# n-lalanne/LDSO

Hardware: AMD Instinct MI355X
Metric: point-residuals/sec per GN iter (7-KF window) + ms/solve; 1/2/4/8 GPU (higher is better)
Workload: dtype f32

## Files before the change

### include/ldso_ba.h

```cpp
#ifndef LDSO_BA_H_
#define LDSO_BA_H_

#include <stddef.h>
#include <stdint.h>

#ifdef __cplusplus
extern "C" {
#endif

#define LDSO_BA_ABI_VERSION 6

#define LDSO_BA_PATTERN_NUM 8
#define LDSO_BA_CPARS 4
#define LDSO_BA_MAX_FRAMES 16
#define LDSO_BA_PRECALC_STRIDE 48
#define LDSO_BA_POINT_STRIDE 24

#define LDSO_BA_RES_IN 0
#define LDSO_BA_RES_OOB 1
#define LDSO_BA_RES_OUTLIER 2

#define LDSO_BA_FLAG_ACTIVE 1u
#define LDSO_BA_FLAG_NEW 2u

// ... 196 lines not shown

int ldso_ba_frame_step(int32_t n_frames, const ldso_ba_frame_state *in, const double *x, ldso_ba_frame_state *out,
                       double *calib_value, const double *calib_value_zero, float *calib_scaled_out,
                       float *c_delta_out);

int ldso_ba_step_canbreak(int32_t n_frames, const double *x, float sum_nid, float num_id, float th_opt_iterations,
                          int32_t *canbreak_out);

int ldso_ba_set_kernel_timing(ldso_ba_ctx *ctx, int32_t enable);

#define LDSO_BA_TUNE_TILED_IMAGES 2
#define LDSO_BA_TUNE_TOP_CHUNK 6
#define LDSO_BA_TUNE_TIMING_MASK 7
#define LDSO_BA_TUNE_ITEM_ORDER 10
#define LDSO_BA_TUNE_SOLVE_EXACT 12
int ldso_ba_set_tuning(ldso_ba_ctx *ctx, int32_t key, int32_t value);
int ldso_ba_get_kernel_times(ldso_ba_ctx *ctx, double *ms, int64_t *counts, int32_t n);
const char *ldso_ba_kernel_name(int32_t i);
int32_t ldso_ba_num_kernels(void);

int ldso_ba_stats(ldso_ba_ctx *ctx, int64_t *device_bytes, int64_t *n_points,
                  int64_t *n_residuals);

#ifdef __cplusplus
}
#endif

#endif
```

### ldso_amd/_lib.py

```python
from __future__ import annotations

import ctypes as C
import os

import numpy as np

HERE = os.path.dirname(os.path.abspath(__file__))
LIB_DIR = os.path.join(HERE, "lib")
LIB_PATH = os.environ.get("LDSO_BA_LIB") or os.path.join(LIB_DIR, "libldso_ba.so")
SYNTH_PATH = os.path.join(LIB_DIR, "libldso_synth.so")

PATTERN_NUM = 8
CPARS = 4
MAX_FRAMES = 16
PRECALC_STRIDE = 48
POINT_STRIDE = 24
RES_IN, RES_OOB, RES_OUTLIER = 0, 1, 2
FLAG_ACTIVE, FLAG_NEW = 1, 2

i32p = C.POINTER(C.c_int32)
f32p = C.POINTER(C.c_float)
f64p = C.POINTER(C.c_double)
i8p = C.POINTER(C.c_int8)
u8p = C.POINTER(C.c_uint8)
# ... 144 lines not shown
    ("ldso_ba_comm_init", C.c_int, [C.c_void_p, C.c_void_p, C.c_int32, C.c_int32]),
    ("ldso_ba_check_settings", C.c_int, [C.c_void_p]),
    ("ldso_ba_default_settings", None, [C.c_void_p]),
    ("ldso_ba_set_settings", C.c_int, [C.c_void_p, C.c_void_p]),
    ("ldso_ba_get_settings", C.c_int, [C.c_void_p, C.c_void_p]),
    ("ldso_ba_optimize", C.c_int, [C.c_void_p, C.c_int32, C.c_void_p, C.c_void_p, f64p, f64p, f64p, f64p, C.c_void_p,
                                   f64p, f32p, i32p, i32p]),
    ("ldso_ba_frame_step", C.c_int, [C.c_int32, C.c_void_p, f64p, C.c_void_p, f64p, f64p, f32p, f32p]),
    ("ldso_ba_step_canbreak", C.c_int, [C.c_int32, f64p, C.c_float, C.c_float, C.c_float, i32p]),
    ("ldso_ba_set_kernel_timing", C.c_int, [C.c_void_p, C.c_int32]),
    ("ldso_ba_set_tuning", C.c_int, [C.c_void_p, C.c_int32, C.c_int32]),
    ("ldso_ba_get_kernel_times", C.c_int, [C.c_void_p, f64p, i64p, C.c_int32]),
    ("ldso_ba_kernel_name", C.c_char_p, [C.c_int32]),
    ("ldso_ba_num_kernels", C.c_int32, []),
    ("ldso_ba_stats", C.c_int, [C.c_void_p, i64p, i64p, i64p]),
    ("ldso_ba_marginalize_frame", C.c_int, [C.c_int32, C.c_int32, f64p, f64p, f64p, f64p, f64p, f64p]),
    ("ldso_ba_ad_ht_delta", C.c_int, [C.c_int32, f64p, f64p, f64p, f32p]),
    ("ldso_ba_calc_m_energy", C.c_int, [C.c_int32, f64p, f64p, f32p, f64p, f64p]),
    ("ldso_ba_calc_l_energy", C.c_int, [C.c_int32, f64p, f64p, f64p, f32p, C.c_int32, f32p, f32p, f64p]),
    ("ldso_ba_load_marginalization", C.c_int, [C.c_void_p, C.c_void_p, C.c_int32, C.POINTER(LdsoBaWindow)]),
    ("ldso_ba_marginalize_points", C.c_int, [C.c_void_p, f32p, f64p, f64p]),
    ("ldso_ba_activate_points", C.c_int, [C.c_void_p, C.c_int32, C.c_int32, C.c_void_p, C.c_int32, C.c_void_p]),
]

f32pp = C.POINTER(f32p)

IMMATURE_DTYPE = np.dtype([("u", "<f4"), ("v", "<f4"), ("idepth_min", "<f4"), ("idepth_max", "<f4"),
                           ("quality", "<f4"), ("energy_th", "<f4"), ("color", "<f4", (8,)),
                           ("weights", "<f4", (8,)), ("grad_h", "<f4", (4,)), ("host", "<i4"),
                           ("last_status", "<i4"), ("last_uv", "<f4", (2,)), ("last_interval", "<f4"),
# ... 69 lines not shown
```

### ldso_amd/context.py

```python
from __future__ import annotations

import ctypes as C

import numpy as np

from . import _lib as L
from .window import Window


class BAContext:
    def __init__(self, device: int = 0):
        self._lib = L.lib()
        h = C.c_void_p()
        L.check(self._lib.ldso_ba_create(int(device), C.byref(h)))
        self._h = h
        self.windows: list[Window] = []
        self._structs = None

    def close(self):
        if getattr(self, "_h", None) is not None and self._h.value:
            self._lib.ldso_ba_destroy(self._h)
            self._h = None

    def __del__(self):
# ... 188 lines not shown
        L.check(self._lib.ldso_ba_unpack_system(self._h))

    def set_tuning(self, key: int, value: int):
        L.check(self._lib.ldso_ba_set_tuning(self._h, int(key), int(value)))

    def set_kernel_timing(self, on: bool):
        L.check(self._lib.ldso_ba_set_kernel_timing(self._h, int(bool(on))))

    def kernel_times(self) -> dict:
        n = int(self._lib.ldso_ba_num_kernels())
        ms = np.zeros(n, np.float64)
        cnt = np.zeros(n, np.int64)
        L.check(self._lib.ldso_ba_get_kernel_times(self._h, L.ptr(ms, L.f64p), L.ptr(cnt, L.i64p), n))
        return {self._lib.ldso_ba_kernel_name(i).decode(): (float(ms[i]), int(cnt[i])) for i in range(n)}

    def stats(self):
        b, p, r = C.c_int64(), C.c_int64(), C.c_int64()
        L.check(self._lib.ldso_ba_stats(self._h, C.byref(b), C.byref(p), C.byref(r)))
        return dict(device_bytes=b.value, points=p.value, residuals=r.value)
```

### ldso_amd/csrc/ldso_ba.hip

```cpp
#include <hip/hip_runtime.h>
#include <hip/hip_ext.h>
#include <rccl/rccl.h>

#include <algorithm>
#include <atomic>
#include <climits>
#include <cmath>
#include <cstdio>
#include <cstdlib>
#include <cstring>
#include <mutex>
#include <string>
#include <vector>

#include "../../include/ldso_ba.h"
#include "../../include/ldso_ct.h"
#include "ldso_ba_internal.h"
#include "se3.h"

using namespace ldso_ba;

namespace {

constexpr int kWave = 64;
// ... 79 lines not shown
    long long frame_stride;
    int tiles_per_row;
    int fix;
    int accumulate;
    const float *ad_ht_delta;
    const int *stop;
    int pass;
    int aff_fix;
};

struct Geo {
    float Ku, Kv, new_idepth;
    float d_xi_x[6], d_xi_y[6], d_C_x[4], d_C_y[4], d_d_x, d_d_y;
};

__device__ inline bool centre_projection(const float *__restrict__ pre, float u, float v, float idz,
                                         float fxl, float fyl, float cxl, float cyl, float wM3, float hM3,
                                         Geo &g) {
#pragma clang fp contract(off)
    const float fxli = 1.0f / fxl, fyli = 1.0f / fyl;
    const float *R0 = pre + 12, *t0 = pre + 21;
    const float K0 = (u + 0 - cxl) * fxli, K1 = (v + 0 - cyl) * fyli;
    float ptp[3];
#pragma unroll
    for (int i = 0; i < 3; i++) ptp[i] = (R0[3 * i] * K0 + R0[3 * i + 1] * K1 + R0[3 * i + 2] * 1.0f) + t0[i] * idz;
    const float drescale = 1.0f / ptp[2];
    g.new_idepth = idz * drescale;
    if (!(drescale > 0)) return false;
    const float uu = ptp[0] * drescale, vv = ptp[1] * drescale;
    g.Ku = uu * fxl + cxl;
    g.Kv = vv * fyl + cyl;
    if (!(g.Ku > 1.1f && g.Kv > 1.1f && g.Ku < wM3 && g.Kv < hM3)) return false;
    g.d_d_x = drescale * (t0[0] - t0[2] * uu) * kScaleIdepth * fxl;
    g.d_d_y = drescale * (t0[1] - t0[2] * vv) * kScaleIdepth * fyl;
    g.d_C_x[2] = drescale * (R0[6] * uu - R0[0]);
    g.d_C_x[3] = fxl * drescale * (R0[7] * uu - R0[1]) * fyli;
// ... 240 lines not shown
    }
}

typedef float f32x4 __attribute__((ext_vector_type(4)));
constexpr int kTopRow = 36;
constexpr int kTermQ = 9;
constexpr int kBoxCols = 9, kBoxBands = 3, kBoxFloats = 112;
static_assert(kBoxFloats >= (kBoxCols * kBoxBands + 1) * 4, "box");
constexpr int kTermStride = 72;
constexpr int kRoundQ = kTermQ;
static_assert(kTermStride >= kRoundQ * 8, "term tables");
constexpr int kTermsOnly = 8 * kTermStride;
constexpr int kTermsPerWave = 8 * kBoxFloats > kTermsOnly ? 8 * kBoxFloats : kTermsOnly;
constexpr int kSumsPerWave = 64 * kSumStride;

__device__ __forceinline__ void top_mfma(float *tab, int lane, bool active, const Geo &g, const PhotoSums &s,
                                         float *slab_item) {
    auto stage = [&](float4 *row) {
        if (active) {
            row[0] = make_float4(g.d_C_x[0], g.d_C_y[0], g.d_C_x[1], g.d_C_y[1]);
            row[1] = make_float4(g.d_C_x[2], g.d_C_y[2], g.d_C_x[3], g.d_C_y[3]);
            row[2] = make_float4(g.d_xi_x[0], g.d_xi_y[0], g.d_xi_x[1], g.d_xi_y[1]);
            row[3] = make_float4(g.d_xi_x[2], g.d_xi_y[2], g.d_xi_x[3], g.d_xi_y[3]);
            row[4] = make_float4(g.d_xi_x[4], g.d_xi_y[4], g.d_xi_x[5], g.d_xi_y[5]);
            row[5] = make_float4(s.JabJIdx_00, s.JabJIdx_01, s.JabJIdx_10, s.JabJIdx_11);
            row[6] = make_float4(s.JI_r0, s.JI_r1, s.Jab2_00, s.Jab2_11);
            row[7] = make_float4(s.Jab2_01, s.Jab_r1, s.Jab_r0, s.rr);
            row[8] = make_float4(s.JIdx2_00, s.JIdx2_10, s.JIdx2_11, 0.f);
        } else {
            const float4 z = make_float4(0.f, 0.f, 0.f, 0.f);
#pragma unroll
            for (int k = 0; k < 9; k++) row[k] = z;
        }
    };
    const int i = lane & 15, kk = lane >> 4;
    const bool geo = i < 10, ind = i >= 13;
    const float a0c = i == 13 ? 1.f : 0.f, a1c = i == 14 ? 1.f : 0.f;
    stage(reinterpret_cast<float4 *>(tab + lane * kTopRow));
    wave_lds_sync();
    f32x4 acc0 = {0.f, 0.f, 0.f, 0.f}, acc1 = {0.f, 0.f, 0.f, 0.f};
    {
        const float *base = tab + kk * kTopRow;
#pragma unroll 4
        for (int m = 0; m < 16; m += 2) {
#pragma unroll
            for (int u = 0; u < 2; u++) {
                const float *rr = base + 4 * (m + u) * kTopRow;
                const float2 p = *reinterpret_cast<const float2 *>(rr + 2 * i);
                const float4 q = *reinterpret_cast<const float4 *>(rr + 32);
                const float A0 = ind ? a0c : p.x, A1 = ind ? a1c : p.y;
                const float B0 = geo ? q.x * p.x + q.y * p.y : p.x;
                const float B1 = geo ? q.y * p.x + q.z * p.y : p.y;
                f32x4 &acc = u ? acc1 : acc0;
                acc = __builtin_amdgcn_mfma_f32_16x16x4f32(A0, B0, acc, 0, 0, 0);
                acc = __builtin_amdgcn_mfma_f32_16x16x4f32(A1, B1, acc, 0, 0, 0);
            }
        }
    }
    wave_lds_sync();
    const f32x4 acc = acc0 + acc1;
#pragma unroll
    for (int v = 0; v < 4; v++) {
        const int r = 4 * kk + v, c = i;
        int slot = -1;
        if (r < 10 && c < 10 && c >= r) slot = r * 10 - r * (r - 1) / 2 + (c - r);
        else if (r < 10 && c >= 10 && c < 13) slot = 55 + 3 * r + (c - 10);
        else if (r == 13 && c >= 13) slot = 85 + (c - 13);
        else if (r == 14 && c >= 13) slot = 88 + (c - 13);
        if (slot >= 0) slab_item[slot] = acc[v];
        else if (r == 15 && c < 5) slab_item[91 + c] = 0.f;
    }
// ... 13 lines not shown
    v = min(v, LDSO_DPP(v, 0xB1));
    v = min(v, LDSO_DPP(v, 0x4E));
    return min(v, LDSO_DPP(v, 0x141));
}
__device__ __forceinline__ int grp8_or(int v) {
    v |= LDSO_DPP(v, 0xB1);
    v |= LDSO_DPP(v, 0x4E);
    return v | LDSO_DPP(v, 0x141);
}
__device__ __forceinline__ float4 ldb4(__amdgpu_buffer_rsrc_t r, unsigned off) {
    typedef int i32x4 __attribute__((ext_vector_type(4)));
    const i32x4 v = __builtin_bit_cast(i32x4, __builtin_amdgcn_raw_buffer_load_b128(r, (int)off, 0, 0));
    return make_float4(__int_as_float(v.x), __int_as_float(v.y), __int_as_float(v.z), __int_as_float(v.w));
}

template <bool kMarg>
__device__ __forceinline__ void phase_a_pieces(int lane, float *lds_terms_w, float *S, const float *pre, int jlimit,
                                               int my_state, float4 my_pd0, float jp_dx, float jp_dy, float da,
                                               float db, __amdgpu_buffer_rsrc_t rsrc, unsigned band, float wM3,
                                               float hM3, int aff_fix) {
#pragma clang fp contract(off)
    const int g = lane >> 3, sl = lane & 7;
    const bool fixA = (aff_fix & 1) != 0, fixB = (aff_fix & 2) != 0;
    const int px = sl == 1 || sl == 6 ? -1 : sl == 2 ? 1 : sl == 3 ? -2 : sl == 5 ? 2 : 0;
    const int py = sl == 0 ? -2 : sl <= 2 ? -1 : sl <= 5 ? 0 : sl == 6 ? 1 : 2;
    const float aff0 = pre[24], aff1 = pre[25], b0a = pre[26];
    float *T = lds_terms_w + g * kTermStride;
    float *box = lds_terms_w + g * kBoxFloats;
    const int nsteps = (jlimit + 7) >> 3;
    constexpr unsigned kOOB = 0x7FFFFFF0u;

    struct Geo8 {
// ... 141 lines not shown
        step(k, cur, nxt);
        if (k + 1 >= nsteps) break;
        step(k + 1, nxt, cur);
    }
    while (wide_steps) {
        const int k = __builtin_ctz(wide_steps);
        wide_steps &= wide_steps - 1;
        geo(k, cur);
        const bool wide = cur.gok && cur.wide;
        float iv[12];
        if (wide) load12(rsrc, band, (int)cur.Ku, (int)cur.Kv, iv);
        terms(k, cur, wide, iv);
    }
}

template <int kImg, bool kMarg>
__global__ __launch_bounds__(256, kLinBlocksPerCu) void k_linearize(LinParams P) {
    static_assert(kImg == 1 || kImg == 3, "image layouts 1 and 3");
    extern __shared__ __attribute__((aligned(16))) float lds_dyn[];
    const int lane = threadIdx.x & 63;
    const int wave = __builtin_amdgcn_readfirstlane(threadIdx.x >> 6);
    float *lds_terms_w = lds_dyn + wave * kWaveLds;
    float *lds_sums_w = lds_terms_w + kTermsPerWave;
    const int nb = P.n_blocks, xcd = blockIdx.x & 7, q8 = nb >> 3, r8 = nb & 7;
    const int lblock = xcd * q8 + min(xcd, r8) + (blockIdx.x >> 3);
    if (lblock * 4 + wave >= P.n_items) return;
    const int itemL = P.item_base + lblock * 4 + wave;
    const int4 it = P.items[itemL];
    if (P.stop && P.pass > P.stop[__builtin_amdgcn_readfirstlane(it.w)]) return;
    const int cnt = it.y & 0xFFFF;
    const bool valid = lane < cnt;
    const int pair = __builtin_amdgcn_readfirstlane(it.z), jlimit = __builtin_amdgcn_readfirstlane(cnt);
    const WinDev &W = P.wins[__builtin_amdgcn_readfirstlane(it.w)];
    const int N = W.N;
    const int h = (pair - W.pair_base) % N, t = (pair - W.pair_base) / N;
    const float *pre = P.precalc + (size_t)pair * LDSO_BA_PRECALC_STRIDE;
    const float th = fmaxf(P.frame_th[W.frame_base + h], P.frame_th[W.frame_base + t]);
    const float wM3 = W.wM3, hM3 = W.hM3;
    const float4 *img = P.img + (size_t)(W.frame_base + t) * P.frame_stride;
    const __amdgpu_buffer_rsrc_t rsrc = frame_rsrc(reinterpret_cast<const float *>(img), P.frame_stride * 16);
    const unsigned band = (unsigned)P.tiles_per_row * 8u * 16u;

    const int r = it.x + lane;
    const int rq = valid ? r : 0;
    int my_state = P.rs_state[rq];
    const int my_slot = P.rs_slot[rq];
    const int my_point = valid ? W.point_base + (my_slot - W.rec_base - (t < h ? t : t - 1) * W.P) : W.point_base;
    uint8_t flags = P.rs_flags[rq];
    float state_energy = P.rs_energy[rq];
    float new_energy = P.rs_newenergy[rq];
    const float4 my_pd0 = *(const float4 *)(P.pt_data + (size_t)my_point * LDSO_BA_POINT_STRIDE);
    {
        const float4 *cw = reinterpret_cast<const float4 *>(P.pt_data + (size_t)my_point * LDSO_BA_POINT_STRIDE + 8);
        float4 v[4];
#pragma unroll
        for (int u = 0; u < 4; u++) v[u] = cw[u];
        float *row = lds_sums_w + lane * kSumStride;
#pragma unroll
        for (int u = 0; u < 4; u++) {
            row[4 * u] = v[u].x;
            row[4 * u + 1] = v[u].y;
            row[4 * u + 2] = v[u].z;
            row[4 * u + 3] = v[u].w;
        }
    }
    if (!valid) my_state = LDSO_BA_RES_OOB;
    float jp_dx = 0.f, jp_dy = 0.f, da = 0.f, db = 0.f;
    if constexpr (kMarg) {
#pragma clang fp contract(off)
        const float *dp = P.ad_ht_delta + (size_t)pair * 8;
        da = dp[6];
        db = dp[7];
        Geo gm;
        if (centre_projection(pre, my_pd0.x, my_pd0.y, my_pd0.w, W.calib[0], W.calib[1], W.calib[2], W.calib[3],
                              wM3, hM3, gm)) {
            const float dd = P.pt_data[(size_t)my_point * LDSO_BA_POINT_STRIDE + 5];
            float x6 = 0.f, y6 = 0.f, x4 = 0.f, y4 = 0.f;
#pragma unroll
            for (int i = 0; i < 6; i++) {
                x6 += gm.d_xi_x[i] * dp[i];
                y6 += gm.d_xi_y[i] * dp[i];
            }
#pragma unroll
            for (int i = 0; i < 4; i++) {
                x4 += gm.d_C_x[i] * W.cdelta[i];
                y4 += gm.d_C_y[i] * W.cdelta[i];
            }
            jp_dx = x6 + x4 + gm.d_d_x * dd;
            jp_dy = y6 + y4 + gm.d_d_y * dd;
        }
    }
// ... 14 lines not shown
        float *T = lds_terms_w + g * (kTermQ * 8);
        float *S = lds_sums_w;
        const int nsteps = (jlimit + 7) >> 3;
        const int tpr2 = P.tiles_per_row;

        struct Stage {
            float Ku, Kv, color, weight;
            float iv[12];
            float3 t00, t10, t01, t11;
            float jx, jy;
            bool gok;
        };
        auto issue = [&](int k, Stage &q) {
            const int j = 8 * k + g;
            const int st = __shfl(my_state, j, kWave);
            const int p = __shfl(my_point, j, kWave);
            const float pu = __shfl(my_pd0.x, j, kWave), pv = __shfl(my_pd0.y, j, kWave),
                        pz = __shfl(my_pd0.z, j, kWave);
            const bool go = j < jlimit && st != LDSO_BA_RES_OOB;
            if constexpr (kMarg) {
                q.jx = __shfl(jp_dx, j, kWave);
                q.jy = __shfl(jp_dy, j, kWave);
            }
            (void)p;
            q.color = S[j * kSumStride + sl];
            q.weight = S[j * kSumStride + 8 + sl];
            const float up = pu + px, vp = pv + py;
            float ptp[3];
#pragma unroll
            for (int i = 0; i < 3; i++)
                ptp[i] = (pre[3 * i] * up + pre[3 * i + 1] * vp + pre[3 * i + 2] * 1.0f) + pre[9 + i] * pz;
            q.Ku = ptp[0] / ptp[2];
            q.Kv = ptp[1] / ptp[2];
            const bool pok = go && q.Ku > 1.1f && q.Kv > 1.1f && q.Ku < wM3 && q.Kv < hM3;
            const unsigned long long m1 = __ballot(pok);
            q.gok = ((m1 >> (8 * g)) & 0xFFull) == 0xFFull;
            const int ix = pok ? (int)q.Ku : 1, iy = pok ? (int)q.Kv : 1;
            if constexpr (kImg == 3) {
                load12(rsrc, band, ix, iy, q.iv);
// ... 61 lines not shown
            }
            wave_lds_sync();
            if (rok) sum8(kTermQ + sl, sl);
            wave_lds_sync();
        };
        Stage A, B;
        issue(0, A);
        for (int k = 0; k < nsteps; k += 2) {
            issue(k + 1, B);
            consume(k, A);
            issue(k + 2, A);
            consume(k + 1, B);
        }
    }

    double energy = 0;
    bool isIN = false, active = false;
    Geo g;
    PhotoSums s;
    if (valid) {
        const int8_t old_state = (int8_t)my_state;
        int8_t new_state = LDSO_BA_RES_OOB;
        float e_wo = -1;
        if (old_state == LDSO_BA_RES_OOB) {
            energy = state_energy;
            st_nt(P.rec_b + my_slot, make_float2(0.f, __builtin_nanf("")));
        } else {
            const float4 pd0 = my_pd0;
            const float *Sr = lds_sums_w + lane * kSumStride;
            s.energy = Sr[0];
// ... 61 lines not shown
        isIN = (new_state == LDSO_BA_RES_IN);
        st_nt(P.rs_newstate + r, new_state);
        st_nt(P.rs_energy_wo + r, e_wo);
    }

    double esum = energy;
#pragma unroll
    for (int m = 32; m >= 1; m >>= 1) esum += __shfl_xor(esum, m, kWave);
    const unsigned long long inmask = __ballot(isIN);
    if (lane == 0) {
        P.item_energy[2 * itemL] = esum;
        P.item_energy[2 * itemL + 1] = (double)__popcll(inmask);
    }
    if ((it.y >> 16) && P.geo_snap && lane < kGeoSnap)
        P.geo_snap[(size_t)pair * kGeoSnap + lane] = lane < 12 ? pre[12 + lane] : W.calib[lane - 12];
    if (!P.accumulate) return;
    wave_lds_sync();
    top_mfma(lds_terms_w, lane, active, g, s, P.top_slab + (size_t)itemL * kTopVals);
}

struct PointParams {
    const int4 *__restrict__ items;
    const WinDev *__restrict__ wins;
    const float *__restrict__ pt_data;
    const int *__restrict__ pt_nres;
    const unsigned long long *__restrict__ pt_tgt;
    const float4 *__restrict__ rec_a;
    const float2 *__restrict__ rec_b;
    const float *__restrict__ precalc;
    float *pt_out;
    float *sc_slab;
    int n_items;
    int item_base;
// ... 1055 lines not shown
                for (int b = 0; b < 2; b++) {
                    if (r0 + a > c0 + b) continue;
                    o[pk_index(4 + 8 * i + r0 + a, 4 + 8 * i + c0 + b, D)] = v[2 * a + b];
                }
        } else {
            const int item = fu - 16, rr = item < 32 ? item >> 2 : item - 32, cc = item & 3;
            double ha = 0;
            for (int st = 0; st < Nm1; st++) ha += CP[(part * 40 + item) * Nm1 + st];
            if (item < 32)
                (top ? HAp : Hsp)[pk_index(cc, 4 + 8 * i + rr, D)] = ha;
            else
                (top ? bAp : bsp)[4 + 8 * i + rr] = ha;
        }
    }
}
__global__ __launch_bounds__(256) void k_stitch_host_sum(const WinDev *__restrict__ wins,
                                                          const int2 *__restrict__ blocks,
                                                          const double *__restrict__ stage, double *sys) {
    const int2 bw = blocks[blockIdx.x];
    const WinDev &W = wins[bw.x];
    const long long n_el = sys_len(W.D), e = (long long)bw.y + threadIdx.x;
    if (e >= n_el) return;
    const double *p = stage + W.stage_base + e;
    double x[kHostStitchMaxN];
#pragma unroll
    for (int h = 0; h < kHostStitchMaxN; h++) x[h] = p[(size_t)min(h, W.N - 1) * n_el];
    double v = 0;
#pragma unroll
    for (int h = 0; h < kHostStitchMaxN; h++)
        if (h < W.N) v += x[h];
    sys[W.sys_base + e] = v;
}

constexpr int kSolveMaxDim = 8 * 11 + 4;
#ifndef LDSO_SOLVE_THREADS
#define LDSO_SOLVE_THREADS 256
#endif
constexpr int kSolveThreads = LDSO_SOLVE_THREADS;
__device__ constexpr int kJacobiRounds[7][3][2] = {
    {{1, 6}, {2, 5}, {3, 4}}, {{0, 2}, {3, 6}, {4, 5}}, {{1, 3}, {0, 4}, {5, 6}}, {{2, 4}, {1, 5}, {0, 6}},
    {{3, 5}, {2, 6}, {0, 1}}, {{4, 6}, {0, 3}, {1, 2}}, {{0, 5}, {1, 4}, {2, 3}}};
constexpr int kXadStride = LDSO_BA_MAX_FRAMES * LDSO_BA_MAX_FRAMES * 8 + 4;
__device__ __forceinline__ void xad_fill(const WinDev &W, const double *xw, const double *__restrict__ adH,
                                         const double *__restrict__ adT, float *o, int tid, int nthreads) {
#pragma clang fp contract(off)
// ... 1573 lines not shown

__global__ void k_tile_image(const float *__restrict__ src, float4 *dst, int w, int h, int tpr2, int hp) {
    const int i = blockIdx.x * blockDim.x + threadIdx.x;
    const int wp = tpr2 * 2;
    if (i >= wp * hp) return;
    const int x = i % wp, y = i / wp;
    float4 v = make_float4(0.f, 0.f, 0.f, 0.f);
    if (x < w && y < h) {
        const float *p = src + 3 * ((size_t)y * w + x);
        v = make_float4(p[0], p[1], p[2], 0.f);
    }
    dst[(((y >> 2) * tpr2 + (x >> 1)) << 3) + ((y & 3) << 1) + (x & 1)] = v;
}

template <bool kMarg>
void launch_linearize(int img_mode, int nb, hipStream_t st, const LinParams &L, hipEvent_t ev_start = nullptr,
                      hipEvent_t ev_stop = nullptr) {
    if (ev_start) {
        if (img_mode == 3)
            hipExtLaunchKernelGGL(k_linearize<3, kMarg>, dim3(nb), dim3(256), kLinLdsBytes, st, ev_start, ev_stop, 0, L);
        else
            hipExtLaunchKernelGGL(k_linearize<1, kMarg>, dim3(nb), dim3(256), kLinLdsBytes, st, ev_start, ev_stop, 0, L);
        return;
    }
    if (img_mode == 3) k_linearize<3, kMarg><<<nb, 256, kLinLdsBytes, st>>>(L);
    else k_linearize<1, kMarg><<<nb, 256, kLinLdsBytes, st>>>(L);
}

std::atomic<unsigned long long> g_alloc_gen{1};
template <typename T>
struct DevBuf {
    T *p = nullptr;
// ... 98 lines not shown
    DevBuf<double> d_prior, d_x, d_ns;
    DevBuf<double> d_ns_nm, d_ns_g;
    std::vector<double> ns_cache;
    int ns_cache_null = -1;
    DevBuf<int> d_pt_win;
    bool marg = false;
    bool host_stitch = false;
    int n_cu = 256;
    const float4 *img_ext = nullptr;
    DevBuf<float> d_adhtd;
    int vec_total = 0;
    size_t sc_smem_max = 0;
    bool timing = false;
    unsigned timing_mask = ~0u;
    int top_chunk = 0;
    int solve_exact = 0;
    int img_mode = 3;
    std::vector<PendingEv> pending;
    std::vector<hipEvent_t> ev_pool;
    double kms[kNumKernels] = {0};
    long long kcount[kNumKernels] = {0};
    std::vector<double> sys_host;
    std::vector<char> sys_valid;
    bool sys_host_valid = false;
    double *pin_sys = nullptr;
    float *pin_xad = nullptr, *pin_step = nullptr;
    size_t pin_sys_n = 0, pin_step_n = 0;
    char *pin_out = nullptr;
    size_t pin_out_n = 0;
    char *pin_map = nullptr, *pin_map_dev = nullptr;
// ... 1217 lines not shown
    L.rs_energy_wo = c->d_rs_energy_wo.p;
    L.rs_center = reinterpret_cast<float *>(c->d_rs_center.p);
    L.center_stride = c->R_tot;
    L.rec_a = c->d_rec_a.p;
    L.rec_b = c->d_rec_b.p;
    L.geo_snap = c->d_geo_snap.p;
    L.top_slab = c->d_top_slab.p;
    L.item_energy = c->d_item_energy.p;
    L.frame_stride = c->frame_stride;
    L.tiles_per_row = c->tiles_per_row;
    L.fix = fix;
    L.accumulate = accumulate;
    L.aff_fix = aff_fix_bits(c);
    L.item_base = 0;
    L.n_items = c->n_top_items;
    L.n_blocks = (L.n_items + 3) / 4;
    PointParams Pp{};
    Pp.items = c->d_sc_items.p;
    Pp.wins = c->d_wins.p;
    Pp.pt_data = c->d_pt_data.p;
    Pp.pt_nres = c->d_pt_nres.p;
    Pp.pt_tgt = c->d_pt_tgt.p;
    Pp.rec_a = c->d_rec_a.p;
    Pp.rec_b = c->d_rec_b.p;
    Pp.precalc = c->d_precalc.p;
    Pp.pt_out = c->d_pt_out.p;
    Pp.sc_slab = c->d_sc_slab.p;
    Pp.shift_prior = c->marg ? 0 : 1;
    Pp.item_base = 0;
    Pp.n_items = c->n_sc_items;
    StitchParams Sp{};
// ... 31 lines not shown
    Sp.n_win = c->n_win;
    int kp_max = 0, n_max = 2;
    for (const WinDev &D : c->wd) {
        kp_max = std::max(kp_max, D.KP);
        n_max = std::max(n_max, D.N);
    }
    Sp.frame_win = c->d_frame_win.p;
    Sp.frame_base = 0;
    Sp.hs_split = Sp.n_win + 2 * c->n_frames <= 2 * c->n_cu ? 1 : 0;
    if (const char *e = std::getenv("LDSO_BA_HS_SPLIT")) Sp.hs_split = e[0] == '1';
    const size_t st_smem = c->host_stitch ? stitch_host_smem_bytes(n_max, &Sp.th_cap)
                                          : stitch_smem_bytes(kp_max, n_max, &Sp.th_cap);
    hipStream_t st = c->stream;
    if (L.n_items > 0) {
        rc = timed_launch_ext(c, 0, st, [&](hipEvent_t a, hipEvent_t b) {
            if (c->marg) launch_linearize<true>(c->img_mode, L.n_blocks, st, L, a, b);
            else launch_linearize<false>(c->img_mode, L.n_blocks, st, L, a, b);
        });
        if (rc) return rc;
    }
    if (accumulate && Pp.n_nid + Pp.n_items > 0) {
        rc = timed_launch(c, 1, st,
                          [&] { k_point_sc<<<Pp.n_nid + Pp.n_items, kScThreads, sc_smem, st>>>(Pp); });
        if (rc) return rc;
    }
    if (c->host_stitch) {
        static std::once_flag once;
        std::call_once(once, [] {
            int th;
            (void)hipFuncSetAttribute((const void *)k_stitch_host, hipFuncAttributeMaxDynamicSharedMemorySize,
                                      (int)stitch_host_smem_bytes(kHostStitchMaxN, &th));
        });
// ... 76 lines not shown
    L.rs_newenergy = c->d_sx_newenergy.p;
    L.rs_energy_wo = c->d_sx_ewo.p;
    L.rs_center = reinterpret_cast<float *>(c->d_sx_center.p);
    L.center_stride = (long long)Rt;
    L.rec_a = c->d_sx_rec_a.p;
    L.rec_b = c->d_sx_rec_b.p;
    L.geo_snap = c->d_sx_geo_snap.p;
    L.top_slab = nullptr;
    L.item_energy = c->d_sx_item.p;
    L.frame_stride = c->frame_stride;
    L.tiles_per_row = c->tiles_per_row;
    L.fix = 0;
    L.accumulate = 0;
    L.item_base = D.top_item_base;
    L.n_items = D.n_top_items;
    L.n_blocks = (L.n_items + 3) / 4;
    rc = timed_launch(c, 0, st, [&] {
        if (c->marg) launch_linearize<true>(c->img_mode, L.n_blocks, st, L);
        else launch_linearize<false>(c->img_mode, L.n_blocks, st, L);
    });
    if (rc) return rc;
    std::vector<int8_t> ns(R);
    std::vector<float> ne(R), ew(R);
    std::vector<float4> ce(R);
    HIP_TRY(hipMemcpyAsync(ns.data(), c->d_sx_newstate.p + b, R, hipMemcpyDeviceToHost, st));
    HIP_TRY(hipMemcpyAsync(ne.data(), c->d_sx_newenergy.p + b, R * sizeof(float), hipMemcpyDeviceToHost, st));
    HIP_TRY(hipMemcpyAsync(ew.data(), c->d_sx_ewo.p + b, R * sizeof(float), hipMemcpyDeviceToHost, st));
    for (int k = 0; k < 4; k++)
        HIP_TRY(hipMemcpy2DAsync(reinterpret_cast<float *>(ce.data()) + k, sizeof(float4),
                                 reinterpret_cast<const float *>(c->d_sx_center.p) + (size_t)k * Rt + b, sizeof(float),
                                 sizeof(float), R, hipMemcpyDeviceToHost, st));
    std::vector<float> jp;
    if (jpjdf && (rc = record_jpjdf(c, win, c->d_sx_rec_a.p, c->d_sx_rec_b.p, c->d_sx_geo_snap.p, jp))) return rc;
    if ((rc = ldso_ba_sync(c))) return rc;
// ... 898 lines not shown
    if (key == LDSO_BA_TUNE_SOLVE_EXACT) {
        if (value != 0 && value != 1) return fail(-1, "solve mode must be 0 (fast) or 1 (exact)");
        c->solve_exact = value;
        return 0;
    }
    if (key == LDSO_BA_TUNE_TIMING_MASK) {
        c->timing_mask = (unsigned)value;
        return 0;
    }
    if (key == LDSO_BA_TUNE_TOP_CHUNK) {
        if (value < 0 || value > 64 || value % 8) return fail(-1, "chunk must be 0 or a multiple of 8 up to 64");
        if (c->n_win) return fail(-1, "chunk size must be chosen before ldso_ba_load");
        c->top_chunk = value;
        return 0;
    }
    return fail(-1, "unknown tuning key");
}

int ldso_ba_set_kernel_timing(ldso_ba_ctx *c, int32_t enable) {
    if (!c) return fail(-1, "null ctx");
    int rc = ldso_ba_sync(c);
    if (rc) return rc;
    c->timing = enable != 0;
    for (int i = 0; i < kNumKernels; i++) {
        c->kms[i] = 0;
        c->kcount[i] = 0;
    }
    while (c->timing && c->ev_pool.size() < 256) {
        hipEvent_t e;
        if (hipEventCreateWithFlags(&e, hipEventDisableSystemFence) != hipSuccess) break;
// ... 4 lines not shown

int ldso_ba_get_kernel_times(ldso_ba_ctx *c, double *ms, int64_t *counts, int32_t n) {
    if (!c) return fail(-1, "null ctx");
    int rc = ldso_ba_sync(c);
    if (rc) return rc;
    for (int i = 0; i < n && i < kNumKernels; i++) {
        if (ms) ms[i] = c->kms[i];
        if (counts) counts[i] = c->kcount[i];
    }
    return 0;
}

const char *ldso_ba_kernel_name(int32_t i) { return (i >= 0 && i < kNumKernels) ? kKernelNames[i] : ""; }
int32_t ldso_ba_num_kernels(void) { return kNumKernels; }

int ldso_ba_stats(ldso_ba_ctx *c, int64_t *device_bytes, int64_t *n_points, int64_t *n_residuals) {
    if (!c) return fail(-1, "null ctx");
    if (device_bytes)
        *device_bytes = (int64_t)(c->d_img.bytes() + c->d_precalc.bytes() + c->d_pt_data.bytes() + c->d_rec_a.bytes() + c->d_rec_b.bytes() +
                                  c->d_top_slab.bytes() + c->d_sc_slab.bytes() + c->d_sys.bytes());
    if (n_points) *n_points = c->P_tot;
    if (n_residuals) *n_residuals = c->R_tot;
    return 0;
}

}
```

Before: 5.432 billion.

## Add two-chunk-per-wave linearize with prefetch, skip idle MFMA, specialize host stitch sum

Restructures the linearize kernel into a per-chunk body plus a chunk-head loader. An optional two-chunks-per-wavefront mode prefetches the second chunk's residual state and point data while the first chunk computes, and it defaults off (lin_chunks=1). It also routes read-only loads through the constant address space and skips the top MFMA accumulation when no lane is active or the chunk is partial. The host-sum stitch kernel gets a switch over frame count to avoid padded loads. The prefetch mode raises register pressure and changes the block count.

```diff
diff --git a/include/ldso_ba.h b/include/ldso_ba.h
--- a/include/ldso_ba.h
+++ b/include/ldso_ba.h
@@ -234,11 +234,14 @@
 #define LDSO_BA_TUNE_TIMING_MASK 7
 #define LDSO_BA_TUNE_ITEM_ORDER 10
 #define LDSO_BA_TUNE_SOLVE_EXACT 12
+#define LDSO_BA_TUNE_LIN_CHUNKS_PER_WAVE 15
 int ldso_ba_set_tuning(ldso_ba_ctx *ctx, int32_t key, int32_t value);
 int ldso_ba_get_kernel_times(ldso_ba_ctx *ctx, double *ms, int64_t *counts, int32_t n);
 const char *ldso_ba_kernel_name(int32_t i);
 int32_t ldso_ba_num_kernels(void);
 
+int ldso_ba_num_chunks(ldso_ba_ctx *ctx, int32_t *n_chunks);
+
 int ldso_ba_stats(ldso_ba_ctx *ctx, int64_t *device_bytes, int64_t *n_points,
                   int64_t *n_residuals);
 
diff --git a/ldso_amd/_lib.py b/ldso_amd/_lib.py
--- a/ldso_amd/_lib.py
+++ b/ldso_amd/_lib.py
@@ -182,6 +182,7 @@
     ("ldso_ba_kernel_name", C.c_char_p, [C.c_int32]),
     ("ldso_ba_num_kernels", C.c_int32, []),
     ("ldso_ba_stats", C.c_int, [C.c_void_p, i64p, i64p, i64p]),
+    ("ldso_ba_num_chunks", C.c_int, [C.c_void_p, i32p]),
     ("ldso_ba_marginalize_frame", C.c_int, [C.c_int32, C.c_int32, f64p, f64p, f64p, f64p, f64p, f64p]),
     ("ldso_ba_ad_ht_delta", C.c_int, [C.c_int32, f64p, f64p, f64p, f32p]),
     ("ldso_ba_calc_m_energy", C.c_int, [C.c_int32, f64p, f64p, f32p, f64p, f64p]),
diff --git a/ldso_amd/context.py b/ldso_amd/context.py
--- a/ldso_amd/context.py
+++ b/ldso_amd/context.py
@@ -226,6 +226,11 @@
         L.check(self._lib.ldso_ba_get_kernel_times(self._h, L.ptr(ms, L.f64p), L.ptr(cnt, L.i64p), n))
         return {self._lib.ldso_ba_kernel_name(i).decode(): (float(ms[i]), int(cnt[i])) for i in range(n)}
 
+    def num_chunks(self) -> int:
+        n = C.c_int32()
+        L.check(self._lib.ldso_ba_num_chunks(self._h, C.byref(n)))
+        return n.value
+
     def stats(self):
         b, p, r = C.c_int64(), C.c_int64(), C.c_int64()
         L.check(self._lib.ldso_ba_stats(self._h, C.byref(b), C.byref(p), C.byref(r)))
diff --git a/ldso_amd/csrc/ldso_ba.hip b/ldso_amd/csrc/ldso_ba.hip
--- a/ldso_amd/csrc/ldso_ba.hip
+++ b/ldso_amd/csrc/ldso_ba.hip
@@ -117,12 +117,13 @@
     float d_xi_x[6], d_xi_y[6], d_C_x[4], d_C_y[4], d_d_x, d_d_y;
 };
 
-__device__ inline bool centre_projection(const float *__restrict__ pre, float u, float v, float idz,
+template <class PreP>
+__device__ inline bool centre_projection(PreP pre, float u, float v, float idz,
                                          float fxl, float fyl, float cxl, float cyl, float wM3, float hM3,
                                          Geo &g) {
 #pragma clang fp contract(off)
     const float fxli = 1.0f / fxl, fyli = 1.0f / fyl;
-    const float *R0 = pre + 12, *t0 = pre + 21;
+    const auto R0 = pre + 12, t0 = pre + 21;
     const float K0 = (u + 0 - cxl) * fxli, K1 = (v + 0 - cyl) * fyli;
     float ptp[3];
 #pragma unroll
@@ -393,8 +394,8 @@
 constexpr int kTermsPerWave = 8 * kBoxFloats > kTermsOnly ? 8 * kBoxFloats : kTermsOnly;
 constexpr int kSumsPerWave = 64 * kSumStride;
 
-__device__ __forceinline__ void top_mfma(float *tab, int lane, bool active, const Geo &g, const PhotoSums &s,
-                                         float *slab_item) {
+__device__ __forceinline__ void top_mfma(float *tab, int lane, int cnt, bool active, const Geo &g,
+                                         const PhotoSums &s, float *slab_item) {
     auto stage = [&](float4 *row) {
         if (active) {
             row[0] = make_float4(g.d_C_x[0], g.d_C_y[0], g.d_C_x[1], g.d_C_y[1]);
@@ -415,25 +416,31 @@
     const int i = lane & 15, kk = lane >> 4;
     const bool geo = i < 10, ind = i >= 13;
     const float a0c = i == 13 ? 1.f : 0.f, a1c = i == 14 ? 1.f : 0.f;
-    stage(reinterpret_cast<float4 *>(tab + lane * kTopRow));
-    wave_lds_sync();
     f32x4 acc0 = {0.f, 0.f, 0.f, 0.f}, acc1 = {0.f, 0.f, 0.f, 0.f};
-    {
+    if (__ballot(active)) {
+        stage(reinterpret_cast<float4 *>(tab + lane * kTopRow));
+        wave_lds_sync();
         const float *base = tab + kk * kTopRow;
-#pragma unroll 4
-        for (int m = 0; m < 16; m += 2) {
+        const int mend = (cnt + 3) >> 2;
+        auto groups2 = [&](int m) {
 #pragma unroll
             for (int u = 0; u < 2; u++) {
                 const float *rr = base + 4 * (m + u) * kTopRow;
                 const float2 p = *reinterpret_cast<const float2 *>(rr + 2 * i);
                 const float4 q = *reinterpret_cast<const float4 *>(rr + 32);
                 const float A0 = ind ? a0c : p.x, A1 = ind ? a1c : p.y;
-                const float B0 = geo ? q.x * p.x + q.y * p.y : p.x;
-                const float B1 = geo ? q.y * p.x + q.z * p.y : p.y;
+                const float B0 = geo ? __builtin_fmaf(q.y, p.y, q.x * p.x) : p.x;
+                const float B1 = geo ? __builtin_fmaf(q.y, p.x, q.z * p.y) : p.y;
                 f32x4 &acc = u ? acc1 : acc0;
                 acc = __builtin_amdgcn_mfma_f32_16x16x4f32(A0, B0, acc, 0, 0, 0);
                 acc = __builtin_amdgcn_mfma_f32_16x16x4f32(A1, B1, acc, 0, 0, 0);
             }
+        };
+        if (mend == 16) {
+#pragma unroll 4
+            for (int m = 0; m < 16; m += 2) groups2(m);
+        } else {
+            for (int m = 0; m < mend; m += 2) groups2(m);
         }
     }
     wave_lds_sync();
@@ -477,8 +484,8 @@
     return make_float4(__int_as_float(v.x), __int_as_float(v.y), __int_as_float(v.z), __int_as_float(v.w));
 }
 
-template <bool kMarg>
-__device__ __forceinline__ void phase_a_pieces(int lane, float *lds_terms_w, float *S, const float *pre, int jlimit,
+template <bool kMarg, class PreP>
+__device__ __forceinline__ void phase_a_pieces(int lane, float *lds_terms_w, float *S, PreP pre, int jlimit,
                                                int my_state, float4 my_pd0, float jp_dx, float jp_dy, float da,
                                                float db, __amdgpu_buffer_rsrc_t rsrc, unsigned band, float wM3,
                                                float hM3, int aff_fix) {
@@ -650,54 +657,78 @@
     }
 }
 
-template <int kImg, bool kMarg>
-__global__ __launch_bounds__(256, kLinBlocksPerCu) void k_linearize(LinParams P) {
-    static_assert(kImg == 1 || kImg == 3, "image layouts 1 and 3");
-    extern __shared__ __attribute__((aligned(16))) float lds_dyn[];
-    const int lane = threadIdx.x & 63;
-    const int wave = __builtin_amdgcn_readfirstlane(threadIdx.x >> 6);
-    float *lds_terms_w = lds_dyn + wave * kWaveLds;
-    float *lds_sums_w = lds_terms_w + kTermsPerWave;
-    const int nb = P.n_blocks, xcd = blockIdx.x & 7, q8 = nb >> 3, r8 = nb & 7;
-    const int lblock = xcd * q8 + min(xcd, r8) + (blockIdx.x >> 3);
-    if (lblock * 4 + wave >= P.n_items) return;
-    const int itemL = P.item_base + lblock * 4 + wave;
-    const int4 it = P.items[itemL];
-    if (P.stop && P.pass > P.stop[__builtin_amdgcn_readfirstlane(it.w)]) return;
+#define LDSO_AS_CONST __attribute__((address_space(4)))
+template <class T>
+__device__ __forceinline__ const LDSO_AS_CONST T *as_const(const T *p) {
+    return (const LDSO_AS_CONST T *)p;
+}
+
+struct ChunkHead {
+    int4 it;
+    int state, slot;
+    uint8_t flags;
+    float energy, newenergy;
+    float4 pd0;
+    float4 cw[4];
+};
+__device__ __forceinline__ int chunk_point(const LinParams &P, const int4 &it, int lane, int slot) {
+    const auto &W = *as_const(P.wins + __builtin_amdgcn_readfirstlane(it.w));
+    const int pair = __builtin_amdgcn_readfirstlane(it.z), N = W.N;
+    const int h = (pair - W.pair_base) % N, t = (pair - W.pair_base) / N;
+    return lane < (it.y & 0xFFFF) ? W.point_base + (slot - W.rec_base - (t < h ? t : t - 1) * W.P) : W.point_base;
+}
+__device__ __forceinline__ void head_load(const LinParams &P, const int4 &it, int lane, ChunkHead &H) {
+    H.it = it;
+    const int rq = lane < (it.y & 0xFFFF) ? it.x + lane : 0;
+    H.state = P.rs_state[rq];
+    H.slot = P.rs_slot[rq];
+    H.flags = P.rs_flags[rq];
+    H.energy = P.rs_energy[rq];
+    H.newenergy = P.rs_newenergy[rq];
+}
+__device__ __forceinline__ void head_point(const LinParams &P, int lane, ChunkHead &H) {
+    const float4 *rec =
+        reinterpret_cast<const float4 *>(P.pt_data + (size_t)chunk_point(P, H.it, lane, H.slot) * LDSO_BA_POINT_STRIDE);
+    H.pd0 = rec[0];
+#pragma unroll
+    for (int u = 0; u < 4; u++) H.cw[u] = rec[2 + u];
+}
+__device__ __forceinline__ bool chunk_stopped(const LinParams &P, const int4 &it) {
+    return P.stop && P.pass > as_const(P.stop)[__builtin_amdgcn_readfirstlane(it.w)];
+}
+
+template <int kImg, bool kMarg, class FA, class FB>
+__device__ __forceinline__ void lin_chunk(const LinParams &P, int lane, float *lds_terms_w, float *lds_sums_w,
+                                          int itemL, const ChunkHead &H, FA after_a, FB after_b) {
+    const int4 it = H.it;
     const int cnt = it.y & 0xFFFF;
     const bool valid = lane < cnt;
     const int pair = __builtin_amdgcn_readfirstlane(it.z), jlimit = __builtin_amdgcn_readfirstlane(cnt);
-    const WinDev &W = P.wins[__builtin_amdgcn_readfirstlane(it.w)];
+    const auto &W = *as_const(P.wins + __builtin_amdgcn_readfirstlane(it.w));
     const int N = W.N;
     const int h = (pair - W.pair_base) % N, t = (pair - W.pair_base) / N;
-    const float *pre = P.precalc + (size_t)pair * LDSO_BA_PRECALC_STRIDE;
-    const float th = fmaxf(P.frame_th[W.frame_base + h], P.frame_th[W.frame_base + t]);
+    const auto pre = as_const(P.precalc + (size_t)pair * LDSO_BA_PRECALC_STRIDE);
+    const float th = fmaxf(as_const(P.frame_th)[W.frame_base + h], as_const(P.frame_th)[W.frame_base + t]);
     const float wM3 = W.wM3, hM3 = W.hM3;
     const float4 *img = P.img + (size_t)(W.frame_base + t) * P.frame_stride;
     const __amdgpu_buffer_rsrc_t rsrc = frame_rsrc(reinterpret_cast<const float *>(img), P.frame_stride * 16);
     const unsigned band = (unsigned)P.tiles_per_row * 8u * 16u;
 
     const int r = it.x + lane;
-    const int rq = valid ? r : 0;
-    int my_state = P.rs_state[rq];
-    const int my_slot = P.rs_slot[rq];
-    const int my_point = valid ? W.point_base + (my_slot - W.rec_base - (t < h ? t : t - 1) * W.P) : W.point_base;
-    uint8_t flags = P.rs_flags[rq];
-    float state_energy = P.rs_energy[rq];
-    float new_energy = P.rs_newenergy[rq];
-    const float4 my_pd0 = *(const float4 *)(P.pt_data + (size_t)my_point * LDSO_BA_POINT_STRIDE);
+    int my_state = H.state;
+    const int my_slot = H.slot;
+    uint8_t flags = H.flags;
+    float state_energy = H.energy;
+    float new_energy = H.newenergy;
+    const float4 my_pd0 = H.pd0;
     {
-        const float4 *cw = reinterpret_cast<const float4 *>(P.pt_data + (size_t)my_point * LDSO_BA_POINT_STRIDE + 8);
-        float4 v[4];
-#pragma unroll
-        for (int u = 0; u < 4; u++) v[u] = cw[u];
         float *row = lds_sums_w + lane * kSumStride;
 #pragma unroll
         for (int u = 0; u < 4; u++) {
-            row[4 * u] = v[u].x;
-            row[4 * u + 1] = v[u].y;
-            row[4 * u + 2] = v[u].z;
-            row[4 * u + 3] = v[u].w;
+            row[4 * u] = H.cw[u].x;
+            row[4 * u + 1] = H.cw[u].y;
+            row[4 * u + 2] = H.cw[u].z;
+            row[4 * u + 3] = H.cw[u].w;
         }
     }
     if (!valid) my_state = LDSO_BA_RES_OOB;
@@ -710,7 +741,7 @@
         Geo gm;
         if (centre_projection(pre, my_pd0.x, my_pd0.y, my_pd0.w, W.calib[0], W.calib[1], W.calib[2], W.calib[3],
                               wM3, hM3, gm)) {
-            const float dd = P.pt_data[(size_t)my_point * LDSO_BA_POINT_STRIDE + 5];
+            const float dd = P.pt_data[(size_t)chunk_point(P, it, lane, my_slot) * LDSO_BA_POINT_STRIDE + 5];
             float x6 = 0.f, y6 = 0.f, x4 = 0.f, y4 = 0.f;
 #pragma unroll
             for (int i = 0; i < 6; i++) {
@@ -755,7 +786,6 @@
         auto issue = [&](int k, Stage &q) {
             const int j = 8 * k + g;
             const int st = __shfl(my_state, j, kWave);
-            const int p = __shfl(my_point, j, kWave);
             const float pu = __shfl(my_pd0.x, j, kWave), pv = __shfl(my_pd0.y, j, kWave),
                         pz = __shfl(my_pd0.z, j, kWave);
             const bool go = j < jlimit && st != LDSO_BA_RES_OOB;
@@ -763,7 +793,6 @@
                 q.jx = __shfl(jp_dx, j, kWave);
                 q.jy = __shfl(jp_dy, j, kWave);
             }
-            (void)p;
             q.color = S[j * kSumStride + sl];
             q.weight = S[j * kSumStride + 8 + sl];
             const float up = pu + px, vp = pv + py;
@@ -855,6 +884,7 @@
         }
     }
 
+    after_a();
     double energy = 0;
     bool isIN = false, active = false;
     Geo g;
@@ -946,9 +976,51 @@
     }
     if ((it.y >> 16) && P.geo_snap && lane < kGeoSnap)
         P.geo_snap[(size_t)pair * kGeoSnap + lane] = lane < 12 ? pre[12 + lane] : W.calib[lane - 12];
+    after_b();
     if (!P.accumulate) return;
     wave_lds_sync();
-    top_mfma(lds_terms_w, lane, active, g, s, P.top_slab + (size_t)itemL * kTopVals);
+    top_mfma(lds_terms_w, lane, jlimit, active, g, s, P.top_slab + (size_t)itemL * kTopVals);
+}
+
+template <int kImg, bool kMarg, int kChunks = 1>
+__global__ __launch_bounds__(256, kLinBlocksPerCu) void k_linearize(LinParams P) {
+    static_assert(kImg == 1 || kImg == 3, "image layouts 1 and 3");
+    static_assert(kChunks == 1 || kChunks == 2, "one or two chunks per wavefront");
+    extern __shared__ __attribute__((aligned(16))) float lds_dyn[];
+    const int lane = threadIdx.x & 63;
+    const int wave = __builtin_amdgcn_readfirstlane(threadIdx.x >> 6);
+    float *lds_terms_w = lds_dyn + wave * kWaveLds;
+    float *lds_sums_w = lds_terms_w + kTermsPerWave;
+    const int nb = P.n_blocks, xcd = blockIdx.x & 7, q8 = nb >> 3, r8 = nb & 7;
+    const int lblock = xcd * q8 + min(xcd, r8) + (blockIdx.x >> 3);
+    const int c0 = lblock * (4 * kChunks) + wave;
+    if (c0 >= P.n_items) return;
+    const auto none = [] {};
+    ChunkHead A;
+    if constexpr (kChunks == 1) {
+        const int4 it = P.items[P.item_base + c0];
+        if (chunk_stopped(P, it)) return;
+        head_load(P, it, lane, A);
+        head_point(P, lane, A);
+        lin_chunk<kImg, kMarg>(P, lane, lds_terms_w, lds_sums_w, P.item_base + c0, A, none, none);
+    } else {
+        const bool haveB = c0 + 4 < P.n_items;
+        const int i0 = P.item_base + c0, i1 = haveB ? i0 + 4 : i0;
+        const int4 itA = P.items[i0], itB = P.items[i1];
+        const bool runA = !chunk_stopped(P, itA), runB = haveB && !chunk_stopped(P, itB);
+        ChunkHead B;
+        if (runA) {
+            head_load(P, itA, lane, A);
+            head_point(P, lane, A);
+            lin_chunk<kImg, kMarg>(P, lane, lds_terms_w, lds_sums_w, i0, A,
+                                   [&] { head_load(P, itB, lane, B); }, [&] { head_point(P, lane, B); });
+            wave_lds_sync();
+        } else if (runB) {
+            head_load(P, itB, lane, B);
+            head_point(P, lane, B);
+        }
+        if (runB) lin_chunk<kImg, kMarg>(P, lane, lds_terms_w, lds_sums_w, i1, B, none, none);
+    }
 }
 
 struct PointParams {
@@ -2034,6 +2106,16 @@
         }
     }
 }
+template <int kN>
+__device__ __forceinline__ double host_sum(const double *__restrict__ p, long long n_el) {
+    double x[kN];
+#pragma unroll
+    for (int h = 0; h < kN; h++) x[h] = p[(size_t)h * n_el];
+    double v = 0;
+#pragma unroll
+    for (int h = 0; h < kN; h++) v += x[h];
+    return v;
+}
 __global__ __launch_bounds__(256) void k_stitch_host_sum(const WinDev *__restrict__ wins,
                                                           const int2 *__restrict__ blocks,
                                                           const double *__restrict__ stage, double *sys) {
@@ -2042,13 +2124,14 @@
     const long long n_el = sys_len(W.D), e = (long long)bw.y + threadIdx.x;
     if (e >= n_el) return;
     const double *p = stage + W.stage_base + e;
-    double x[kHostStitchMaxN];
-#pragma unroll
-    for (int h = 0; h < kHostStitchMaxN; h++) x[h] = p[(size_t)min(h, W.N - 1) * n_el];
-    double v = 0;
-#pragma unroll
-    for (int h = 0; h < kHostStitchMaxN; h++)
-        if (h < W.N) v += x[h];
+    double v;
+    switch (W.N) {
+#define LDSO_HS_SUM(n) case n: v = host_sum<n>(p, n_el); break;
+        LDSO_HS_SUM(1) LDSO_HS_SUM(2) LDSO_HS_SUM(3) LDSO_HS_SUM(4) LDSO_HS_SUM(5) LDSO_HS_SUM(6)
+        LDSO_HS_SUM(7) LDSO_HS_SUM(8) LDSO_HS_SUM(9) LDSO_HS_SUM(10)
+#undef LDSO_HS_SUM
+        default: v = host_sum<kHostStitchMaxN>(p, n_el); break;
+    }
     sys[W.sys_base + e] = v;
 }
 
@@ -3652,8 +3735,20 @@
 }
 
 template <bool kMarg>
-void launch_linearize(int img_mode, int nb, hipStream_t st, const LinParams &L, hipEvent_t ev_start = nullptr,
+void launch_linearize(int img_mode, int chunks, hipStream_t st, LinParams L, hipEvent_t ev_start = nullptr,
                       hipEvent_t ev_stop = nullptr) {
+    const bool two = !kMarg && img_mode == 3 && chunks == 2;
+    const int nb = L.n_blocks = (L.n_items + (two ? 7 : 3)) / (two ? 8 : 4);
+    if constexpr (!kMarg) {
+        if (two) {
+            if (ev_start)
+                hipExtLaunchKernelGGL((k_linearize<3, false, 2>), dim3(nb), dim3(256), kLinLdsBytes, st, ev_start,
+                                      ev_stop, 0, L);
+            else
+                k_linearize<3, false, 2><<<nb, 256, kLinLdsBytes, st>>>(L);
+            return;
+        }
+    }
     if (ev_start) {
         if (img_mode == 3)
             hipExtLaunchKernelGGL(k_linearize<3, kMarg>, dim3(nb), dim3(256), kLinLdsBytes, st, ev_start, ev_stop, 0, L);
@@ -3782,6 +3877,7 @@
     bool timing = false;
     unsigned timing_mask = ~0u;
     int top_chunk = 0;
+    int lin_chunks = 1;
     int solve_exact = 0;
     int img_mode = 3;
     std::vector<PendingEv> pending;
@@ -5029,7 +5125,6 @@
     L.aff_fix = aff_fix_bits(c);
     L.item_base = 0;
     L.n_items = c->n_top_items;
-    L.n_blocks = (L.n_items + 3) / 4;
     PointParams Pp{};
     Pp.items = c->d_sc_items.p;
     Pp.wins = c->d_wins.p;
@@ -5091,8 +5186,8 @@
     hipStream_t st = c->stream;
     if (L.n_items > 0) {
         rc = timed_launch_ext(c, 0, st, [&](hipEvent_t a, hipEvent_t b) {
-            if (c->marg) launch_linearize<true>(c->img_mode, L.n_blocks, st, L, a, b);
-            else launch_linearize<false>(c->img_mode, L.n_blocks, st, L, a, b);
+            if (c->marg) launch_linearize<true>(c->img_mode, c->lin_chunks, st, L, a, b);
+            else launch_linearize<false>(c->img_mode, c->lin_chunks, st, L, a, b);
         });
         if (rc) return rc;
     }
@@ -5199,10 +5294,9 @@
     L.accumulate = 0;
     L.item_base = D.top_item_base;
     L.n_items = D.n_top_items;
-    L.n_blocks = (L.n_items + 3) / 4;
     rc = timed_launch(c, 0, st, [&] {
-        if (c->marg) launch_linearize<true>(c->img_mode, L.n_blocks, st, L);
-        else launch_linearize<false>(c->img_mode, L.n_blocks, st, L);
+        if (c->marg) launch_linearize<true>(c->img_mode, c->lin_chunks, st, L);
+        else launch_linearize<false>(c->img_mode, c->lin_chunks, st, L);
     });
     if (rc) return rc;
     std::vector<int8_t> ns(R);
@@ -6131,6 +6225,11 @@
         c->top_chunk = value;
         return 0;
     }
+    if (key == LDSO_BA_TUNE_LIN_CHUNKS_PER_WAVE) {
+        if (value != 1 && value != 2) return fail(-1, "chunks per wavefront must be 1 or 2");
+        c->lin_chunks = value;
+        return 0;
+    }
     return fail(-1, "unknown tuning key");
 }
 
@@ -6165,6 +6264,12 @@
 const char *ldso_ba_kernel_name(int32_t i) { return (i >= 0 && i < kNumKernels) ? kKernelNames[i] : ""; }
 int32_t ldso_ba_num_kernels(void) { return kNumKernels; }
 
+int ldso_ba_num_chunks(ldso_ba_ctx *c, int32_t *n_chunks) {
+    if (!c || !n_chunks) return fail(-1, "bad arguments");
+    *n_chunks = c->n_top_items;
+    return 0;
+}
+
 int ldso_ba_stats(ldso_ba_ctx *c, int64_t *device_bytes, int64_t *n_points, int64_t *n_residuals) {
     if (!c) return fail(-1, "null ctx");
     if (device_bytes)
```

Result: no change. 5.468 billion (median of 3 runs) (+0.7%).
